# GeertRoks/AMD-Versal-phylogenetic-likelihood-function

Measured on AMD Instinct MI355X. Metric: PLF sites/sec (4-state DNA, fp64) at 1/2/4/8 MI355X; % HBM roofline, higher is better.
Workload: dtype f64

## Files before the change

amd-versal-phylogenetic-likelihood-function_amd/csrc/plf_psr.hip:

```cpp
#include <hip/hip_runtime.h>

#include <algorithm>
#include <cstdint>

#define PLFX_SECONDARY_TU
#include "plf_psr.hpp"
#include "plf_kernels.hpp"
#include "plf_launch.hpp"

namespace plfx {
namespace {

using dev::kBlock;
static_assert(kBlockThreads == kBlock, "block size mismatch");
static_assert(dev::kMaxBatch == kMaxBatch && dev::kWsWords == kWsWords, "batch constants");
using bools = among<false, true>;

template <typename T>
constexpr int kNodeU = sizeof(T) == 8 ? 2 : 4;
constexpr int kStreamU = 4;

template <typename T, bool T1, bool T2>
hipError_t launch_plf_psr_t(const NodeDescH *nodes, int count, const void *EV, const uint8_t *rate_cat, int ncat,
                            const int32_t *wgt, int64_t n, const void *tipvec, unsigned long long *ws,
                            int max_blocks, hipStream_t s) {
  constexpr int U = kNodeU<T>;
  const auto p = pack<dev::NodeBatch>(nodes, count, [](const NodeDescH &d) { return d.scaler_sum != nullptr; });
  static int cache[2] = {0, 0};
  auto go = [&](auto kSum) {
    auto kernel = &dev::plf_psr_kernel<T, U, kSum(), T1, T2>;
    const int64_t gx = grid_x((const void *)kernel, cache[kSum() ? 1 : 0], n, kBlock * U, count, max_blocks);
    return launch(kernel, dim3((unsigned)gx, (unsigned)count), kBlock, s, p.b, (const T *)EV, rate_cat, ncat, wgt,
                  n, ws, (const T *)tipvec);
  };
  return p.any_sum ? go(std::true_type{}) : go(std::false_type{});
}

template <typename T, int kTips>
hipError_t launch_plf_psr_triples_t(const TripleDescH *t, int count, const void *EV, const uint8_t *rate_cat,
                                    int ncat, const int32_t *wgt, int64_t n, const void *tipvec,
                                    unsigned long long *ws, int max_blocks, hipStream_t s) {
  constexpr int U = kNodeU<T>;
  static_assert(dev::PsrTripleLds<T, kTips>::kValues * sizeof(T) <= 160 * 1024, "LDS of a gfx950 workgroup");
  const auto p = pack<dev::TripleBatch>(t, count, [](const TripleDescH &d) { return d.ssa || d.ssb || d.ssp; });
  static int cache[2] = {0, 0};
  auto go = [&](auto kSum) {
    auto kernel = &dev::plf_psr_triple_kernel<T, U, kSum(), kTips>;
    const int64_t gx = grid_x((const void *)kernel, cache[kSum() ? 1 : 0], n, kBlock * U, count, max_blocks);
    return launch(kernel, dim3((unsigned)gx, (unsigned)count), kBlock, s, p.b, (const T *)EV, rate_cat, ncat, wgt,
                  n, ws, (const T *)tipvec);
  };
  return p.any_sum ? go(std::true_type{}) : go(std::false_type{});
}

template <typename K>
int64_t lnl_grid(K kernel, int &cache, int64_t n, int max_blocks) {
  return std::min<int64_t>(grid_x((const void *)kernel, cache, n, kBlock * kStreamU, 1, max_blocks), kLnlMaxGrid);
}

template <typename T>
int64_t edge_deriv_psr_grid(int64_t n, int max_blocks) {
  static int cache = 0;
  return lnl_grid(&dev::edge_deriv_psr_kernel<T, kStreamU>, cache, n, max_blocks);
}

template <typename T>
constexpr int kSumtabSitesPerTrip = kBlock * 4 / (4 * (int)sizeof(T) / 16);

}

hipError_t launch_plf_psr(int dtype, int tips, const NodeDescH *nodes, int count, const void *EV,
                          const uint8_t *rate_cat, int ncat, const int32_t *wgt, int64_t n, const void *tipvec,
                          unsigned long long *ws, int max_blocks, hipStream_t s) {
  if (count < 1 || count > kMaxBatch || ncat < 1 || ncat > dev::kPsrMaxCats || n < 1) return hipErrorInvalidValue;
  return dispatch(
      [&](auto k64, auto kT1, auto kT2) {
        return launch_plf_psr_t<real_t<k64()>, kT1(), kT2()>(nodes, count, EV, rate_cat, ncat, wgt, n, tipvec, ws,
                                                            max_blocks, s);
      },
      bools{dtype == 1}, bools{(tips & 1) != 0}, bools{(tips & 2) != 0});
}

hipError_t launch_plf_psr_triples(int dtype, int tips, const TripleDescH *t, int count, const void *EV,
                                  const uint8_t *rate_cat, int ncat, const int32_t *wgt, int64_t n,
                                  const void *tipvec, unsigned long long *ws, int max_blocks, hipStream_t s) {
  static_assert(dev::kMaxTriples == kMaxTriples, "triple batch size");
  if (count < 1 || count > kMaxTriples || ncat < 1 || ncat > dev::kPsrMaxCats || n < 1) return hipErrorInvalidValue;
  return dispatch(
      [&](auto k64, auto kTips) {
        return launch_plf_psr_triples_t<real_t<k64()>, kTips()>(t, count, EV, rate_cat, ncat, wgt, n, tipvec, ws,
                                                                max_blocks, s);
      },
      bools{dtype == 1}, among<0, 1, 2>{tips});
}

hipError_t launch_root_lnl_psr(int dtype, const void *x, int64_t n, const double *freq, const int32_t *wgt,
                               const int64_t *scaler_sums, int nsums, double *partials,
                               unsigned long long *ticket, double *out, double *site_lnl, int max_blocks,
                               hipStream_t s) {
  return dispatch(
      [&](auto k64) {
        using T = real_t<k64()>;
        static int cache = 0;
        auto kernel = &dev::root_lnl_psr_kernel<T, kStreamU>;
        const int64_t gx = lnl_grid(kernel, cache, n, max_blocks);
// ... 78 lines not shown
```

amd-versal-phylogenetic-likelihood-function_amd/csrc/plf_psr.hpp:

```cpp
#pragma once
#include <hip/hip_runtime.h>
#include <cstdint>
#include <type_traits>

#include "plf_edge.hpp"

namespace plfx {
namespace dev {

constexpr int kPsrMaxCats = 32;

template <typename T>
struct PsrRow {
  static constexpr int kChunk = 16 / (int)sizeof(T);
  static constexpr int kStride = 16 + kChunk;
  using V = std::conditional_t<sizeof(T) == 8, f64x2, f32x4>;
};

__device__ __forceinline__ int psr_cat(int byte, int ncat) { return byte < ncat ? byte : ncat - 1; }

template <typename T>
__device__ __forceinline__ void psr_stage(const T *__restrict__ P, int ncat, T *sP) {
  for (int i = threadIdx.x; i < ncat * 16; i += kBlock) sP[(i >> 4) * PsrRow<T>::kStride + (i & 15)] = P[i];
}

template <typename T>
__device__ __forceinline__ void psr_tip_table(const T *__restrict__ P, const T *__restrict__ tv, int ncat,
                                              T *tab) {
  for (int i = threadIdx.x; i < ncat * 64; i += kBlock) {
    const int c = i >> 6, code = (i >> 2) & 15, k = i & 3;
    T v = T(0);
#pragma unroll
    for (int l = 0; l < 4; l++) v += (tv ? tv[code * 4 + l] : T((code >> l) & 1)) * P[c * 16 + k * 4 + l];
    tab[i] = v;
  }
}

template <typename T, int N>
__device__ __forceinline__ void psr_lds_row(const T *row, T (&m)[N]) {
  using V = typename PsrRow<T>::V;
  constexpr int kChunk = PsrRow<T>::kChunk;
  static_assert(N % kChunk == 0, "whole chunks");
  const V *r = reinterpret_cast<const V *>(row);
#pragma unroll
  for (int j = 0; j < N / kChunk; j++) {
    const V v = r[j];
#pragma unroll
    for (int e = 0; e < kChunk; e++) m[j * kChunk + e] = v[e];
  }
}

template <typename T, int U, bool kSum, bool T1, bool T2>
__global__ void __launch_bounds__(kBlock)
plf_psr_kernel(const NodeBatch nodes, const T *__restrict__ EV, const uint8_t *__restrict__ rate_cat, int ncat,
               const int32_t *__restrict__ wgt, int64_t n, unsigned long long *ws,
               const T *__restrict__ tipvec) {
  constexpr int kStride = PsrRow<T>::kStride;
  const NodeDesc &d = nodes.d[blockIdx.y];
  const T *__restrict__ x1 = static_cast<const T *>(d.x1);
  const T *__restrict__ x2 = static_cast<const T *>(d.x2);
  const uint8_t *__restrict__ tip1 = static_cast<const uint8_t *>(d.x1);
  const uint8_t *__restrict__ tip2 = static_cast<const uint8_t *>(d.x2);
  T *__restrict__ x3 = static_cast<T *>(d.x3);
  uint8_t *__restrict__ scaler = d.scaler;
  unsigned long long *wsn = ws + (size_t)blockIdx.y * kWsWords;

  __shared__ __attribute__((aligned(16))) T sL[T1 ? 4 : kPsrMaxCats * kStride];
  __shared__ __attribute__((aligned(16))) T sR[T2 ? 4 : kPsrMaxCats * kStride];
  __shared__ __attribute__((aligned(16))) T tab1[T1 ? kPsrMaxCats * 64 : 4];
  __shared__ __attribute__((aligned(16))) T tab2[T2 ? kPsrMaxCats * 64 : 4];
  if constexpr (T1) psr_tip_table<T>(static_cast<const T *>(d.left), tipvec, ncat, tab1);
  else psr_stage<T>(static_cast<const T *>(d.left), ncat, sL);
  if constexpr (T2) psr_tip_table<T>(static_cast<const T *>(d.right), tipvec, ncat, tab2);
  else psr_stage<T>(static_cast<const T *>(d.right), ncat, sR);
  __syncthreads();

  T E[16];
#pragma unroll
  for (int i = 0; i < 16; i++) E[i] = EV[i];
  const T m = Num<T>::minlik();

  long long acc = 0;
  const int64_t stride = (int64_t)gridDim.x * (kBlock * U);
  const int64_t nlast = n - 1;
  for (int64_t base = (int64_t)blockIdx.x * (kBlock * U); base < n; base += stride) {
    T a[U][4], b[U][4];
    int cat[U], k1[U], k2[U], w[U];
#pragma unroll
    for (int u = 0; u < U; u++) {
      const int64_t site = base + u * kBlock + threadIdx.x;
      const int64_t ld = site < n ? site : nlast;
      cat[u] = rate_cat[ld];
      if constexpr (T1) k1[u] = tip1[ld] & 15;
      else Num<T>::template load4<true>(x1 + ld * 4, a[u]);
      if constexpr (T2) k2[u] = tip2[ld] & 15;
      else Num<T>::template load4<true>(x2 + ld * 4, b[u]);
      if (kSum) w[u] = wgt_at(wgt, ld, ws);
    }
#pragma unroll
    for (int u = 0; u < U; u++) {
      const int64_t site = base + u * kBlock + threadIdx.x;
      const int c = psr_cat(cat[u], ncat);
      T u1[4], u2[4];
      if constexpr (T1) {
        psr_lds_row<T, 4>(tab1 + (c * 16 + k1[u]) * 4, u1);
      } else {
        T PL[16];
        psr_lds_row<T, 16>(sL + c * kStride, PL);
#pragma unroll
        for (int k = 0; k < 4; k++) {
          u1[k] = T(0);
#pragma unroll
          for (int l = 0; l < 4; l++) u1[k] += a[u][l] * PL[k * 4 + l];
        }
      }
      if constexpr (T2) {
        psr_lds_row<T, 4>(tab2 + (c * 16 + k2[u]) * 4, u2);
      } else {
        T PR[16];
        psr_lds_row<T, 16>(sR + c * kStride, PR);
#pragma unroll
        for (int k = 0; k < 4; k++) {
          u2[k] = T(0);
#pragma unroll
          for (int l = 0; l < 4; l++) u2[k] += b[u][l] * PR[k * 4 + l];
        }
      }
      T o[4] = {T(0), T(0), T(0), T(0)};
#pragma unroll
      for (int k = 0; k < 4; k++) {
        const T p = u1[k] * u2[k];
#pragma unroll
        for (int l = 0; l < 4; l++) o[l] += p * E[4 * k + l];
      }
      const bool sc = (Num<T>::abs(o[0]) < m) && (Num<T>::abs(o[1]) < m) && (Num<T>::abs(o[2]) < m) &&
                      (Num<T>::abs(o[3]) < m);
#pragma unroll
// ... 46 lines not shown
    const T p = u1[k] * u2[k];
#pragma unroll
    for (int l = 0; l < 4; l++) o[l] += p * E[4 * k + l];
  }
  const bool sc = (Num<T>::abs(o[0]) < m) && (Num<T>::abs(o[1]) < m) && (Num<T>::abs(o[2]) < m) &&
                  (Num<T>::abs(o[3]) < m);
#pragma unroll
  for (int l = 0; l < 4; l++) {
    const T s = o[l] * Num<T>::two32();
    o[l] = sc ? s : o[l];
  }
  return sc;
}

template <typename T, int kTips>
struct PsrTripleLds {
  static constexpr int kMat = kPsrMaxCats * PsrRow<T>::kStride;
  static constexpr int kTab = kPsrMaxCats * 64;
  static constexpr int kSide1 = kTips >= 1 ? kTab : kMat, kSide2 = kTips == 2 ? kTab : kMat;
  static constexpr int kValues = 2 * kSide1 + 2 * kSide2 + 2 * kMat;
};

template <typename T, int U, bool kSum, int kTips>
__global__ void __launch_bounds__(kBlock)
plf_psr_triple_kernel(const TripleBatch tb, const T *__restrict__ EV, const uint8_t *__restrict__ rate_cat,
                      int ncat, const int32_t *__restrict__ wgt, int64_t n, unsigned long long *ws,
                      const T *__restrict__ tipvec) {
  constexpr bool T1 = kTips >= 1, T2 = kTips == 2;
  constexpr int kStride = PsrRow<T>::kStride;
  using Lds = PsrTripleLds<T, kTips>;
  const TripleDesc &d = tb.d[blockIdx.y];

  __shared__ __attribute__((aligned(16))) T lds[Lds::kValues];
  T *const sA1 = lds, *const sB1 = sA1 + Lds::kSide1, *const sA2 = sB1 + Lds::kSide1;
  T *const sB2 = sA2 + Lds::kSide2, *const sLP = sB2 + Lds::kSide2, *const sRP = sLP + Lds::kMat;
  if constexpr (T1) {
    psr_tip_table<T>((const T *)d.la, tipvec, ncat, sA1);
    psr_tip_table<T>((const T *)d.lb, tipvec, ncat, sB1);
  } else {
    psr_stage<T>((const T *)d.la, ncat, sA1);
    psr_stage<T>((const T *)d.lb, ncat, sB1);
  }
  if constexpr (T2) {
    psr_tip_table<T>((const T *)d.ra, tipvec, ncat, sA2);
    psr_tip_table<T>((const T *)d.rb, tipvec, ncat, sB2);
  } else {
    psr_stage<T>((const T *)d.ra, ncat, sA2);
    psr_stage<T>((const T *)d.rb, ncat, sB2);
  }
  psr_stage<T>((const T *)d.lp, ncat, sLP);
  psr_stage<T>((const T *)d.rp, ncat, sRP);
  __syncthreads();

  T E[16];
#pragma unroll
  for (int i = 0; i < 16; i++) E[i] = EV[i];
  const T m = Num<T>::minlik();
  const T *__restrict__ xa1 = (const T *)d.a1, *__restrict__ xa2 = (const T *)d.a2;
  const T *__restrict__ xb1 = (const T *)d.b1, *__restrict__ xb2 = (const T *)d.b2;
  const uint8_t *__restrict__ ta1 = (const uint8_t *)d.a1, *__restrict__ ta2 = (const uint8_t *)d.a2;
  const uint8_t *__restrict__ tb1 = (const uint8_t *)d.b1, *__restrict__ tb2 = (const uint8_t *)d.b2;
  T *__restrict__ xa = (T *)d.xa, *__restrict__ xb = (T *)d.xb, *__restrict__ xp = (T *)d.xp;

  long long accA = 0, accB = 0, accP = 0;
  const int64_t stride = (int64_t)gridDim.x * (kBlock * U);
  const int64_t nlast = n - 1;
  for (int64_t base = (int64_t)blockIdx.x * (kBlock * U); base < n; base += stride) {
    T va1[U][4], va2[U][4], vb1[U][4], vb2[U][4];
    int cat[U], ka1[U], ka2[U], kb1[U], kb2[U], w[U];
#pragma unroll
    for (int u = 0; u < U; u++) {
      const int64_t site = base + u * kBlock + threadIdx.x;
      const int64_t ld = site < n ? site : nlast;
      cat[u] = rate_cat[ld];
      if constexpr (T1) {
        ka1[u] = ta1[ld] & 15;
        kb1[u] = tb1[ld] & 15;
      } else {
        Num<T>::template load4<true>(xa1 + ld * 4, va1[u]);
        Num<T>::template load4<true>(xb1 + ld * 4, vb1[u]);
      }
      if constexpr (T2) {
        ka2[u] = ta2[ld] & 15;
        kb2[u] = tb2[ld] & 15;
      } else {
        Num<T>::template load4<true>(xa2 + ld * 4, va2[u]);
        Num<T>::template load4<true>(xb2 + ld * 4, vb2[u]);
      }
      if (kSum) w[u] = wgt_at(wgt, ld, ws);
    }
#pragma unroll
    for (int u = 0; u < U; u++) {
      const int64_t site = base + u * kBlock + threadIdx.x;
      const int c = psr_cat(cat[u], ncat);
      T oA[4], oB[4], oP[4];
      const bool sA = psr_site<T, T1, T2>(va1[u], va2[u], T1 ? sA1 + (c * 16 + ka1[u]) * 4 : sA1 + c * kStride,
                                          T2 ? sA2 + (c * 16 + ka2[u]) * 4 : sA2 + c * kStride, E, m, oA);
      const bool sB = psr_site<T, T1, T2>(vb1[u], vb2[u], T1 ? sB1 + (c * 16 + kb1[u]) * 4 : sB1 + c * kStride,
                                          T2 ? sB2 + (c * 16 + kb2[u]) * 4 : sB2 + c * kStride, E, m, oB);
      const bool sP = psr_site<T, false, false>(oA, oB, sLP + c * kStride, sRP + c * kStride, E, m, oP);
      if (site < n) {
        Num<T>::store4_nt(xa + site * 4, oA);
        Num<T>::store4_nt(xb + site * 4, oB);
        Num<T>::store4_nt(xp + site * 4, oP);
        if (d.sa) d.sa[site] = (uint8_t)sA;
        if (d.sb) d.sb[site] = (uint8_t)sB;
        if (d.sp) d.sp[site] = (uint8_t)sP;
        if (kSum) {
          accA += sA ? (long long)w[u] : 0ll;
          accB += sB ? (long long)w[u] : 0ll;
          accP += sP ? (long long)w[u] : 0ll;
        }
      }
    }
  }
  if constexpr (kSum)
    block_ticket_sum3(accA, accB, accP, ws + (size_t)blockIdx.y * 3 * kWsWords, d.ssa, d.ssb, d.ssp);
}

// ... 226 lines not shown
```

amd-versal-phylogenetic-likelihood-function_amd/csrc/plfx_api.hip:

```cpp
#include <hip/hip_runtime.h>

#include <cmath>
#include <cstdarg>
#include <cstdio>
#include <cstring>
#include <algorithm>
#include <new>
#include <string>
#include <mutex>
#include <vector>

#include "../../include/plfx.h"
#include "edge_newton.hpp"
#include "plf_kernels.hpp"
#include "psr_edge_lower.hpp"
#include "psr_lower.hpp"
#include "stream_ws.hpp"
#include "testbench.hpp"
#include "trav_lower.hpp"
#include "trav_plan.hpp"

constexpr int kHostChunksMax = 16;

using plfx::StreamWs;
using plfx::aligned16;
using plfx::clv_bytes_of;
using plfx::overlap;
constexpr int kWsPool = PLFX_WS_POOL;

struct plfx_ctx {
  int device = 0;
  hipStream_t stream = nullptr;
  int max_blocks = 0;
  int node_segments = -1;
  int streams = 1;
  int fuse = 3;
  int psr_fuse = 0;
  bool lazy_tables = false;
  plfx::WsPool wss{hipStreamPerThread};
  std::vector<void *> ws_blocks;
  uint8_t *tt_codes = nullptr;
  double *edge_buf = nullptr;
  int sched[PLFX_SCHED_COUNTS] = {};
  plfx::LaunchList lowered;
  plfx::PsrLaunchList psr_lowered;
  plfx::PsrEdgeLaunchList psr_edges_lowered;
  void *d_buf = nullptr;
  size_t d_cap = 0;
  hipStream_t d2h_stream = nullptr;
  hipEvent_t chunk_done[kHostChunksMax] = {};
  std::string err;
  mutable std::recursive_mutex mu;
};

namespace {

struct DeviceGuard {
  int prev = -1;
  explicit DeviceGuard(int dev) {
    if (hipGetDevice(&prev) != hipSuccess) prev = -1;
    if (prev != dev) (void)hipSetDevice(dev);
    else prev = -1;
  }
  ~DeviceGuard() {
    if (prev >= 0) (void)hipSetDevice(prev);
  }
  DeviceGuard(const DeviceGuard &) = delete;
  DeviceGuard &operator=(const DeviceGuard &) = delete;
};

#define PLFX_BIND(ctx)                                              \
  if (!(ctx)) return PLFX_ERR_INVALID;                              \
  std::lock_guard<std::recursive_mutex> plfx_lock_((ctx)->mu);      \
  DeviceGuard plfx_guard_((ctx)->device)

constexpr size_t kWsRegions = std::max({(size_t)plfx::kMaxBatch, (size_t)7 * plfx::kMaxSeptets,
                                        (size_t)plfx::kDeepNodes, (size_t)plfx::kDeepQueueRegion + 1});
constexpr size_t kWsBytes = kWsRegions * plfx::kWsWords * sizeof(unsigned long long);
constexpr size_t kLnlPartialBytes = 3 * (size_t)plfx::kLnlMaxGrid * sizeof(double);
constexpr size_t kEdgeBufBytes = 4 * sizeof(double);
constexpr size_t kLnlTicketBytes = plfx::kWsWords * sizeof(unsigned long long);
constexpr size_t kEdgeStateRegionBytes = (size_t)plfx::kMaxBatch * plfx::kEdgeStateBytes;

int fail(plfx_ctx *ctx, int code, const char *fmt, ...) {
  if (ctx) {
    char buf[512];
    va_list ap;
    va_start(ap, fmt);
    vsnprintf(buf, sizeof buf, fmt, ap);
    va_end(ap);
// ... 357 lines not shown
                                       c.n, tipvec, ws, ctx->max_blocks, s);
    if (e != hipSuccess) return hip_fail(ctx, e, triples ? "plf_psr level-pair launch" : "plf_psr launch");
  }
  return PLFX_OK;
}

int plan_call(plfx_ctx *ctx, const plfx_trav_op *ops, int nops, const uint8_t *const *tips, int nslots, int npmats,
              int states, int fuse, plfx::TravPlan *plan) {
  std::vector<unsigned char> tip_mask;
  if (nops > 0 && tips)
    for (int sl = 0; sl < nslots; sl++) tip_mask.push_back(tips[sl] != nullptr);
  std::string err;
  if (plfx::plan_traversal(ops, nops, nslots, npmats, tip_mask.empty() ? nullptr : tip_mask.data(), states, fuse,
                           plan, &err) != PLFX_OK)
    return fail(ctx, PLFX_ERR_INVALID, "%s", err.c_str());
  return PLFX_OK;
}

int publish_sched(plfx_ctx *ctx, const plfx::TravPlan &plan, int launches) {
  static_assert(PLFX_SCHED_COUNTS == 7, "the plan's six counts, then the launches");
  std::copy(plan.counts, plan.counts + 6, ctx->sched);
  ctx->sched[6] = launches;
  return PLFX_OK;
}

int check_sumtable_args(plfx_ctx *ctx, const uint8_t *tip1, const void *x1, const void *x2, int64_t n,
                        const void *tipvec, const void *sumtab, size_t clv_bytes) {
  if ((tip1 != nullptr) == (x1 != nullptr))
    return fail(ctx, PLFX_ERR_INVALID, "side 1 needs exactly one of tip / CLV");
  if (tip1 && !tipvec)
    return fail(ctx, PLFX_ERR_INVALID, "a coded side needs tipvec (the default 0/1 table is not in eigen coordinates)");
  if (n < 0) return fail(ctx, PLFX_ERR_INVALID, "n < 0 (%lld)", (long long)n);
  if (n == 0) return PLFX_OK;
  if (!x2 || !sumtab) return fail(ctx, PLFX_ERR_INVALID, "null CLV / sum table pointer");
  if ((x1 && !aligned16(x1)) || !aligned16(x2) || !aligned16(sumtab))
    return fail(ctx, PLFX_ERR_INVALID, "CLV pointers must be 16-byte aligned");
  if (overlap(sumtab, clv_bytes, tip1 ? (const void *)tip1 : x1, tip1 ? (size_t)n : clv_bytes) ||
      overlap(sumtab, clv_bytes, x2, clv_bytes))
    return fail(ctx, PLFX_ERR_INVALID, "sumtab may not overlap x1/x2");
  return PLFX_OK;
}

int check_sums_args(plfx_ctx *ctx, const char *who, bool required, const int64_t *scaler_sums, int nsums) {
  if (!required || nsums < 0 || (nsums > 0 && !scaler_sums))
    return fail(ctx, PLFX_ERR_INVALID, "bad %s arguments", who);
  return PLFX_OK;
}

bool env_settings(plfx_ctx *ctx) {
  if (const char *env = std::getenv("PLFX_MAX_BLOCKS")) {
    int v = std::atoi(env);
    if (v > 0) ctx->max_blocks = v;
  }
  if (const char *env = std::getenv("PLFX_FUSE")) ctx->fuse = ctx->psr_fuse = std::atoi(env);
  if (const char *env = std::getenv("PLFX_NODE_SEGMENTS")) {
    if (!std::strcmp(env, "1")) ctx->node_segments = 1;
    else if (!std::strcmp(env, "0")) ctx->node_segments = 0;
    else if (!std::strcmp(env, "-1") || !std::strcmp(env, "auto") || !*env) ctx->node_segments = -1;
    else return false;
  }
  const char *env = std::getenv("PLFX_STREAMS");
  if (env && *env) {
    static_assert(PLFX_STREAMS_MAX <= 9, "PLFX_STREAMS is parsed as one digit");
    const int v = (env[0] >= '1' && env[0] <= '0' + PLFX_STREAMS_MAX && !env[1]) ? env[0] - '0' : 0;
    if (!v) return false;
    ctx->streams = v;
  }
  return true;
}

int check_edge_args(plfx_ctx *ctx, int dtype, int states, const void *sumtab, int64_t n,
                           const double *eigen, const double *rates, int ncat) {
  if (int rc = check_dtype(ctx, dtype); rc != PLFX_OK) return rc;
  if (states != 4 && states != 20) return fail(ctx, PLFX_ERR_UNSUPPORTED, "edge: states=%d not built (4, 20)", states);
  if (ncat != 4) return fail(ctx, PLFX_ERR_UNSUPPORTED, "edge: ncat=%d not built (4)", ncat);
  if (n < 0) return fail(ctx, PLFX_ERR_INVALID, "n < 0 (%lld)", (long long)n);
  if (!eigen || !rates || (n > 0 && !sumtab)) return fail(ctx, PLFX_ERR_INVALID, "edge: null sum table / eigen / rates");
  if (!aligned16(sumtab)) return fail(ctx, PLFX_ERR_INVALID, "the sum table must be 16-byte aligned");
  return PLFX_OK;
}

int check_psr_edge_args(plfx_ctx *ctx, int dtype, const void *sumtab, int64_t n, const double *eigen,
                        const double *rates, int ncat, const uint8_t *rate_cat) {
  if (int rc = check_dtype(ctx, dtype); rc != PLFX_OK) return rc;
  if (ncat < 1 || ncat > PLFX_PSR_MAX_CATS)
    return fail(ctx, PLFX_ERR_INVALID, "psr edge: ncat=%d outside 1..%d", ncat, PLFX_PSR_MAX_CATS);
  if (n < 0) return fail(ctx, PLFX_ERR_INVALID, "n < 0 (%lld)", (long long)n);
  if (!eigen || !rates || (n > 0 && (!sumtab || !rate_cat)))
    return fail(ctx, PLFX_ERR_INVALID, "psr edge: null sum table / eigen / rates / rate_cat");
  if (!aligned16(sumtab)) return fail(ctx, PLFX_ERR_INVALID, "the sum table must be 16-byte aligned");
  return PLFX_OK;
}

template <typename Eval>
int edge_newton_loop(plfx_ctx *ctx, const char *who, double t0, double tmin, double tmax, int max_evals,
                     double *t_opt, double *out3_host, int *evals, hipStream_t s, Eval eval) {
  if (!t_opt) return fail(ctx, PLFX_ERR_INVALID, "%s: null t_opt", who);
  plfx::EdgeNewton step(t0, tmin, tmax, max_evals);
  if (!step.valid())
    return fail(ctx, PLFX_ERR_INVALID, "%s: needs 0 < tmin <= t0 <= tmax and max_evals >= 1", who);
  if (capturing(s))
    return fail(ctx, PLFX_ERR_INVALID, "%s waits for every evaluation: not on a capturing stream", who);
  double *d_t = ctx->edge_buf, *d_out = ctx->edge_buf + 1;
  double t = 0.0, out[3] = {0.0, 0.0, 0.0};
  for (bool more = true; more;) {
    t = step.t();
    PLFX_HIP(ctx, hipMemcpyAsync(d_t, &t, sizeof t, hipMemcpyHostToDevice, s));
// ... 441 lines not shown
}

int plfx_edge_optimize_dev(plfx_ctx *ctx, int dtype, int states, const void *const *sumtabs, int nedges,
                           int64_t n, const double *eigen, const double *rates, int ncat, const double *catw,
                           const int32_t *wgt, const double *t0, double tmin, double tmax, int max_evals,
                           double *t_opt, double *out3, int32_t *evals, void *stream) {
  PLFX_BIND(ctx);
  if (nedges < 1 || !sumtabs) return fail(ctx, PLFX_ERR_INVALID, "edge_optimize_dev: nedges=%d / null sumtabs", nedges);
  for (int j = 0; j < nedges; j++) {
    if (!sumtabs[j]) return fail(ctx, PLFX_ERR_INVALID, "edge_optimize_dev: sum table %d is null", j);
    if (int rc = check_edge_args(ctx, dtype, states, sumtabs[j], n, eigen, rates, ncat); rc != PLFX_OK) return rc;
  }
  if (!t0 || !t_opt) return fail(ctx, PLFX_ERR_INVALID, "edge_optimize_dev: null t0 / t_opt");
  if (!(tmin > 0.0 && tmin <= tmax && std::isfinite(tmax)) || max_evals < 1 || max_evals > PLFX_EDGE_MAX_EVALS)
    return fail(ctx, PLFX_ERR_INVALID, "edge_optimize_dev: needs 0 < tmin <= tmax < inf and 1 <= max_evals <= %d",
                PLFX_EDGE_MAX_EVALS);
  hipStream_t s = pick(stream);
  PLFX_WS(ctx, s, w);
  for (int g = 0; g < nedges; g += plfx::kMaxBatch) {
    const int c = std::min(nedges - g, plfx::kMaxBatch);
    hipError_t e = plfx::launch_edge_optimize(dtype, states, sumtabs + g, c, n, eigen, rates, catw, wgt, t0 + g, tmin,
                                              tmax, max_evals, w->edge_state, w->lnl_partials, w->ws, t_opt + g,
                                              out3 ? out3 + 3 * (size_t)g : nullptr, evals ? evals + g : nullptr,
                                              ctx->max_blocks, s);
    if (e != hipSuccess) return hip_fail(ctx, e, "edge_optimize_dev launch");
  }
  return PLFX_OK;
}


int plfx_plf_psr_dev(plfx_ctx *ctx, int dtype, const plfx_psr_node *nodes, int count, const void *EV,
                     int64_t n, const uint8_t *rate_cat, int ncat, const int32_t *wgt, const void *tipvec,
                     void *stream) {
  PLFX_BIND(ctx);
  static_assert(PLFX_PSR_MAX_CATS <= 256, "a category is one byte");
  std::string err;
  const plfx::PsrCall call{dtype, n, ncat, EV, rate_cat};
  if (plfx::lower_psr(call, nodes, count, &ctx->psr_lowered, &err) != PLFX_OK)
    return fail(ctx, PLFX_ERR_INVALID, "%s", err.c_str());
  hipStream_t s = pick(stream);
  if (n == 0) return zero_node_sums(ctx, s, nodes, count);
  PLFX_WS(ctx, s, w);
  return execute_psr(ctx, ctx->psr_lowered, call, wgt, tipvec, s, w->ws);
}

int plfx_traverse_psr(plfx_ctx *ctx, int dtype, const plfx_trav_op *ops, int nops, void *const *clv,
                      const uint8_t *const *tips, int nslots, const void *pmats, int npmats,
                      const void *EV, int64_t n, const uint8_t *rate_cat, int ncat, const int32_t *wgt,
                      uint8_t *const *scalers, int64_t *scaler_sums, const void *tipvec, void *stream) {
  PLFX_BIND(ctx);
  for (int &c : ctx->sched) c = 0;
  if (nops < 0 || (nops > 0 && (!ops || !clv))) return fail(ctx, PLFX_ERR_INVALID, "bad traverse_psr arguments");
  plfx::TravPlan plan;
  if (int rc = plan_call(ctx, ops, nops, tips, nslots, npmats, 4, std::min(ctx->psr_fuse, 1), &plan); rc != PLFX_OK)
    return rc;
  const plfx::TravArrays arrays{ops, nops, clv, tips, pmats, scalers, scaler_sums};
  const plfx::PsrCall call{dtype, n, ncat, EV, rate_cat};
  std::string err;
  if (plfx::lower_psr_traversal(plan, arrays, call, &ctx->psr_lowered, &err) != PLFX_OK)
    return fail(ctx, PLFX_ERR_INVALID, "%s", err.c_str());
  hipStream_t s = pick(stream);
  if (n == 0 || nops == 0) {
    const int rc = zero_sums(ctx, s, scaler_sums, nops);
    return rc != PLFX_OK ? rc : publish_sched(ctx, plan, 0);
  }
  PLFX_WS(ctx, s, w);
  if (int rc = execute_psr(ctx, ctx->psr_lowered, call, wgt, tipvec, s, w->ws); rc != PLFX_OK) return rc;
  return publish_sched(ctx, plan, ctx->psr_lowered.launches());
}

int plfx_root_lnl_psr(plfx_ctx *ctx, int dtype, const void *x, int64_t n, const double *freq,
                      const int32_t *wgt, const int64_t *scaler_sums, int nsums, double *out_lnl,
                      double *site_lnl, void *stream) {
  PLFX_BIND(ctx);
  if (int rc = check_dtype(ctx, dtype); rc != PLFX_OK) return rc;
  if (int rc = check_sums_args(ctx, "root_lnl_psr", out_lnl && n >= 0 && (n == 0 || x), scaler_sums, nsums);
      rc != PLFX_OK)
    return rc;
  if (!aligned16(x)) return fail(ctx, PLFX_ERR_INVALID, "the CLV must be 16-byte aligned");
  hipStream_t s = pick(stream);
  if (n == 0) {
    const int rc = zero_sums(ctx, s, out_lnl, 1);
    if (rc != PLFX_OK || nsums == 0) return rc;
  }
  PLFX_WS(ctx, s, w);
  hipError_t e = plfx::launch_root_lnl_psr(dtype, x, n, freq, wgt, scaler_sums, nsums, w->lnl_partials,
                                           w->lnl_ticket, out_lnl, site_lnl, ctx->max_blocks, s);
  if (e != hipSuccess) return hip_fail(ctx, e, "root_lnl_psr launch");
  return PLFX_OK;
}

int plfx_edge_sumtable_psr(plfx_ctx *ctx, int dtype, const uint8_t *tip1, const void *x1, const void *x2,
                           int64_t n, const void *tipvec, void *sumtab, void *stream) {
  PLFX_BIND(ctx);
  if (int rc = check_dtype(ctx, dtype); rc != PLFX_OK) return rc;
  const int rc = check_sumtable_args(ctx, tip1, x1, x2, n, tipvec, sumtab, plfx::psr_clv_bytes(dtype, n));
  if (rc != PLFX_OK || n == 0) return rc;
  hipError_t e = plfx::launch_edge_sumtable_psr(dtype, tip1 != nullptr, tip1 ? (const void *)tip1 : x1, x2, n,
                                                tipvec, sumtab, ctx->max_blocks, pick(stream));
  if (e != hipSuccess) return hip_fail(ctx, e, "edge_sumtable_psr launch");
  return PLFX_OK;
}

int plfx_edge_derivatives_psr(plfx_ctx *ctx, int dtype, const void *sumtab, int64_t n, const double *eigen,
                              const double *rates, int ncat, const uint8_t *rate_cat, const int32_t *wgt,
                              const double *t, const int64_t *scaler_sums, int nsums, double *out3,
                              double *site_lnl, void *stream) {
  PLFX_BIND(ctx);
// ... 71 lines not shown
```

amd-versal-phylogenetic-likelihood-function_amd/csrc/psr_lower.cpp:

```cpp
#include "psr_lower.hpp"

#include <algorithm>
#include <cstdint>
#include <cstdio>
#include <utility>

namespace plfx {
namespace {

struct Prefix {
  const char *call, *unit;
};
constexpr Prefix kBatch{"psr", "psr node"}, kTrav{"psr traverse", "psr traverse op"};

int refuse(PsrLaunchList *out, std::string *err, const Prefix &who, const char *what, int i = -1) {
  out->clear();
  if (err) {
    char buf[160];
    if (i >= 0) std::snprintf(buf, sizeof buf, "%s %d: %s", who.unit, i, what);
    else std::snprintf(buf, sizeof buf, "%s: %s", who.call, what);
    *err = buf;
  }
  return PLFX_ERR_INVALID;
}

const char *check_call(const PsrCall &c, const char *own, bool none, bool *run) {
  *run = false;
  if (c.dtype != PLFX_F32 && c.dtype != PLFX_F64) return "bad dtype";
  if (c.ncat < 1 || c.ncat > PLFX_PSR_MAX_CATS) return "ncat outside 1..PLFX_PSR_MAX_CATS";
  if (c.n < 0) return "n < 0";
  if (own) return own;
  if (c.n == 0 || none) return nullptr;
  if (!c.EV || !c.rate_cat) return "null EV / rate_cat";
  *run = true;
  return nullptr;
}

const char *check_node(const plfx_node &d, bool t1, bool t2, size_t cb, size_t n) {
  if (!d.x1 || !d.x2 || !d.x3 || !d.left || !d.right) return "null CLV / tip / matrix pointer";
  if ((!t1 && !aligned16(d.x1)) || (!t2 && !aligned16(d.x2)) || !aligned16(d.x3))
    return "CLV pointers must be 16-byte aligned";
  if (overlap(d.x3, cb, d.x1, t1 ? n : cb) || overlap(d.x3, cb, d.x2, t2 ? n : cb))
    return "the parent may not overlap a child it reads";
  return nullptr;
}

void add_nodes(PsrLaunchList *out, int level, const std::vector<NodeDescH> (&nb)[4]) {
  for (int k = 0; k < 4; k++) {
    const int first = (int)out->nodes.size(), count = (int)nb[k].size();
    out->nodes.insert(out->nodes.end(), nb[k].begin(), nb[k].end());
    for (int i = 0; i < count; i += kMaxBatch)
      out->items.push_back(PsrLaunch{kPsrNodes, level, k, first + i, std::min(kMaxBatch, count - i)});
  }
}

}

int lower_psr(const PsrCall &call, const plfx_psr_node *nodes, int count, PsrLaunchList *out, std::string *err) {
  out->clear();
  bool run;
  if (const char *f = check_call(call, count < 1 || !nodes ? "needs count >= 1 nodes" : nullptr, false, &run))
    return refuse(out, err, kBatch, f);
  if (!run) return PLFX_OK;

  const size_t cb = psr_clv_bytes(call.dtype, call.n);
  std::vector<NodeDescH> nb[4];
  for (int i = 0; i < count; i++) {
    const plfx_psr_node &d = nodes[i];
    if ((d.tip1 != nullptr) == (d.x1 != nullptr)) return refuse(out, err, kBatch, "child 1 needs exactly one of tip / CLV", i);
    if ((d.tip2 != nullptr) == (d.x2 != nullptr)) return refuse(out, err, kBatch, "child 2 needs exactly one of tip / CLV", i);
    const bool t1 = d.tip1 != nullptr, t2 = d.tip2 != nullptr;
    const plfx_node nd{t1 ? (const void *)d.tip1 : d.x1, t2 ? (const void *)d.tip2 : d.x2, d.x3, d.left, d.right,
                       d.scaler, d.scaler_sum};
    if (const char *f = check_node(nd, t1, t2, cb, (size_t)call.n)) return refuse(out, err, kBatch, f, i);
    nb[(t1 ? 1 : 0) | (t2 ? 2 : 0)].push_back(node_desc(nd));
  }
  add_nodes(out, 0, nb);
  return PLFX_OK;
}

int lower_psr_traversal(const TravPlan &plan, const TravArrays &t, const PsrCall &call, PsrLaunchList *out,
                        std::string *err) {
  out->clear();
  bool run;
  if (const char *f = check_call(call, t.nops < 0 || (t.nops > 0 && !t.ops) ? "null ops" : nullptr, t.nops == 0, &run))
    return refuse(out, err, kTrav, f);
  if (!run) return PLFX_OK;
  if (!t.pmats || !t.clv) return refuse(out, err, kTrav, "null pmats / clv");
  if ((int)plan.level.size() != t.nops || (int)plan.fused.size() != t.nops)
    return refuse(out, err, kTrav, "the plan is not this op list's");

  const size_t cb = psr_clv_bytes(call.dtype, call.n), tb = (size_t)call.n;
  const size_t mat_bytes = (size_t)call.ncat * 16 * (call.dtype == PLFX_F32 ? 4 : 8);
  for (int j = 0; j < t.nops; j++) {
    const OpNode d = op_node(t, mat_bytes, j);
    if (const char *f = check_node(d.nd, d.t1, d.t2, cb, tb)) return refuse(out, err, kTrav, f, j);
  }
  for (const TravGroup &g : plan.groups) {
    if (g.kind != kTravTriple || g.ops.size() != 3 || g.tips < 0 || g.tips > 2)
      return refuse(out, err, kTrav, "the plan holds a fused group other than a level pair");
    const OpNode A = op_node(t, mat_bytes, g.ops[0]), B = op_node(t, mat_bytes, g.ops[1]);
    const void *outs[3] = {A.nd.x3, B.nd.x3, t.clv[t.ops[g.ops[2]].parent]};
    const std::pair<const void *, size_t> leaves[4] = {{A.nd.x1, A.t1 ? tb : cb}, {A.nd.x2, A.t2 ? tb : cb},
                                                       {B.nd.x1, B.t1 ? tb : cb}, {B.nd.x2, B.t2 ? tb : cb}};
    for (int i = 0; i < 3; i++) {
      for (int k = i + 1; k < 3; k++)
        if (overlap(outs[i], cb, outs[k], cb))
          return refuse(out, err, kTrav, "two outputs of a fused level pair overlap", g.ops[2]);
// ... 36 lines not shown
```

amd-versal-phylogenetic-likelihood-function_amd/csrc/psr_lower.hpp:

```cpp
#pragma once
#include <string>
#include <vector>

#include "../../include/plfx.h"
#include "plf_desc.hpp"
#include "trav_lower.hpp"
#include "trav_plan.hpp"

namespace plfx {

struct PsrCall {
  int dtype;
  int64_t n;
  int ncat;
  const void *EV;
  const uint8_t *rate_cat;
};

enum PsrLaunchKind {
  kPsrNodes,
  kPsrTriples,
};

struct PsrLaunch {
  int kind;
  int level;
  int tips;
  int first, count;
};

struct PsrLaunchList {
  std::vector<PsrLaunch> items;
  std::vector<NodeDescH> nodes;
  std::vector<TripleDescH> triples;
  void clear() {
    items.clear();
    nodes.clear();
    triples.clear();
  }
  int launches() const { return (int)items.size(); }
};

inline size_t psr_clv_bytes(int dtype, int64_t n) {
  return (size_t)(n > 0 ? n : 0) * 4 * (dtype == PLFX_F32 ? 4 : 8);
}

int lower_psr(const PsrCall &call, const plfx_psr_node *nodes, int count, PsrLaunchList *out, std::string *err);

int lower_psr_traversal(const TravPlan &plan, const TravArrays &t, const PsrCall &call, PsrLaunchList *out,
                        std::string *err);

}
```

Baseline: 16.52 billion.

## Split fp64 PSR sites across lane pairs and size-gate level-pair fusion

For fp64, each site is now handled by two lanes, each owning two of the four states. Partial sums are exchanged through DPP quad moves, and loads and stores become 16-byte nontemporal vectors. Unroll and grid sizing change as well: a short-unroll variant is used when it covers n, and resident blocks per CU are capped. PSR level-pair fusion is now on by default above a site-count threshold, aiming for better coalescing, more parallelism and fewer launches, at the cost of cross-lane shuffles and a more complex launch path.

```diff
diff --git a/amd-versal-phylogenetic-likelihood-function_amd/csrc/plf_psr.hip b/amd-versal-phylogenetic-likelihood-function_amd/csrc/plf_psr.hip
--- a/amd-versal-phylogenetic-likelihood-function_amd/csrc/plf_psr.hip
+++ b/amd-versal-phylogenetic-likelihood-function_amd/csrc/plf_psr.hip
@@ -16,41 +16,57 @@
 static_assert(dev::kMaxBatch == kMaxBatch && dev::kWsWords == kWsWords, "batch constants");
 using bools = among<false, true>;
 
-template <typename T>
-constexpr int kNodeU = sizeof(T) == 8 ? 2 : 4;
+constexpr int kNodeU = 4, kTripleU = 4, kShortU = 2;
 constexpr int kStreamU = 4;
 
+template <typename T, int kLongU, bool kShort, int kPerCu, typename KernelOf, typename Batch>
+hipError_t launch_psr_stream(KernelOf kernel_of, const Packed<Batch> &p, int count, const void *EV,
+                             const uint8_t *rate_cat, int ncat, const int32_t *wgt, int64_t n, const void *tipvec,
+                             unsigned long long *ws, int max_blocks, hipStream_t s) {
+  static int cache[2][2] = {{0, 0}, {0, 0}};
+  auto with = [&](auto kSum) {
+    auto grid = [&](auto kU) {
+      const void *kernel = (const void *)kernel_of(kSum, kU);
+      int &resident = cache[kSum() ? 1 : 0][kU() == kLongU ? 0 : 1];
+      if (kPerCu > 0 && !resident)
+        resident = std::min(resident_blocks(kernel, kBlock, 2, resident), kPerCu * cu_count());
+      return grid_x(kernel, resident, n, dev::PsrMap<T>::kBlockSites * kU(), count, max_blocks);
+    };
+    auto go = [&](auto kU, int64_t gx) {
+      return launch(kernel_of(kSum, kU), dim3((unsigned)gx, (unsigned)count), kBlock, s, p.b, (const T *)EV, rate_cat,
+                    ncat, wgt, n, ws, (const T *)tipvec);
+    };
+    constexpr std::integral_constant<int, kShortU> kS{};
+    constexpr std::integral_constant<int, kLongU> kL{};
+    if constexpr (kShort) {
+      const int64_t gx = grid(kS);
+      if (gx * (dev::PsrMap<T>::kBlockSites * kShortU) >= n) return go(kS, gx);
+    }
+    return go(kL, grid(kL));
+  };
+  return p.any_sum ? with(std::true_type{}) : with(std::false_type{});
+}
+
+constexpr int kNodeBlocksPerCu64 = 3;
 template <typename T, bool T1, bool T2>
 hipError_t launch_plf_psr_t(const NodeDescH *nodes, int count, const void *EV, const uint8_t *rate_cat, int ncat,
                             const int32_t *wgt, int64_t n, const void *tipvec, unsigned long long *ws,
                             int max_blocks, hipStream_t s) {
-  constexpr int U = kNodeU<T>;
   const auto p = pack<dev::NodeBatch>(nodes, count, [](const NodeDescH &d) { return d.scaler_sum != nullptr; });
-  static int cache[2] = {0, 0};
-  auto go = [&](auto kSum) {
-    auto kernel = &dev::plf_psr_kernel<T, U, kSum(), T1, T2>;
-    const int64_t gx = grid_x((const void *)kernel, cache[kSum() ? 1 : 0], n, kBlock * U, count, max_blocks);
-    return launch(kernel, dim3((unsigned)gx, (unsigned)count), kBlock, s, p.b, (const T *)EV, rate_cat, ncat, wgt,
-                  n, ws, (const T *)tipvec);
-  };
-  return p.any_sum ? go(std::true_type{}) : go(std::false_type{});
+  return launch_psr_stream<T, kNodeU, sizeof(T) == 8, sizeof(T) == 8 ? kNodeBlocksPerCu64 : 0>(
+      [](auto kSum, auto kU) { return &dev::plf_psr_kernel<T, kU(), kSum(), T1, T2>; }, p, count, EV, rate_cat, ncat,
+      wgt, n, tipvec, ws, max_blocks, s);
 }
 
 template <typename T, int kTips>
 hipError_t launch_plf_psr_triples_t(const TripleDescH *t, int count, const void *EV, const uint8_t *rate_cat,
                                     int ncat, const int32_t *wgt, int64_t n, const void *tipvec,
                                     unsigned long long *ws, int max_blocks, hipStream_t s) {
-  constexpr int U = kNodeU<T>;
   static_assert(dev::PsrTripleLds<T, kTips>::kValues * sizeof(T) <= 160 * 1024, "LDS of a gfx950 workgroup");
   const auto p = pack<dev::TripleBatch>(t, count, [](const TripleDescH &d) { return d.ssa || d.ssb || d.ssp; });
-  static int cache[2] = {0, 0};
-  auto go = [&](auto kSum) {
-    auto kernel = &dev::plf_psr_triple_kernel<T, U, kSum(), kTips>;
-    const int64_t gx = grid_x((const void *)kernel, cache[kSum() ? 1 : 0], n, kBlock * U, count, max_blocks);
-    return launch(kernel, dim3((unsigned)gx, (unsigned)count), kBlock, s, p.b, (const T *)EV, rate_cat, ncat, wgt,
-                  n, ws, (const T *)tipvec);
-  };
-  return p.any_sum ? go(std::true_type{}) : go(std::false_type{});
+  return launch_psr_stream<T, kTripleU, true, 0>(
+      [](auto kSum, auto kU) { return &dev::plf_psr_triple_kernel<T, kU(), kSum(), kTips>; }, p, count, EV, rate_cat,
+      ncat, wgt, n, tipvec, ws, max_blocks, s);
 }
 
 template <typename K>
diff --git a/amd-versal-phylogenetic-likelihood-function_amd/csrc/plf_psr.hpp b/amd-versal-phylogenetic-likelihood-function_amd/csrc/plf_psr.hpp
--- a/amd-versal-phylogenetic-likelihood-function_amd/csrc/plf_psr.hpp
+++ b/amd-versal-phylogenetic-likelihood-function_amd/csrc/plf_psr.hpp
@@ -48,6 +48,65 @@
 #pragma unroll
     for (int e = 0; e < kChunk; e++) m[j * kChunk + e] = v[e];
   }
+}
+
+template <typename T>
+struct PsrMap {
+  static constexpr int kLanes = sizeof(T) == 8 ? 2 : 1;
+  static constexpr int kBlockSites = kBlock / kLanes;
+};
+
+constexpr int kPairSwap = 1 | (0 << 2) | (3 << 4) | (2 << 6);
+
+__device__ __forceinline__ void psr_pair_ev(const double *__restrict__ EV, int h, double (&E)[4][2]) {
+#pragma unroll
+  for (int k = 0; k < 4; k++)
+#pragma unroll
+    for (int t = 0; t < 2; t++) E[k][t] = EV[4 * k + 2 * h + t];
+}
+
+__device__ __forceinline__ void psr_pair_ump(const f64x2 x, const double *rows, double (&u)[2]) {
+  double P[8];
+  psr_lds_row<double, 8>(rows, P);
+  const double x0 = dpp_f64<kQuadEven>(x.x), x1 = dpp_f64<kQuadEven>(x.y);
+  const double x2 = dpp_f64<kQuadOdd>(x.x), x3 = dpp_f64<kQuadOdd>(x.y);
+#pragma unroll
+  for (int kk = 0; kk < 2; kk++) {
+    double v = 0.0;
+    v += x0 * P[kk * 4 + 0];
+    v += x1 * P[kk * 4 + 1];
+    v += x2 * P[kk * 4 + 2];
+    v += x3 * P[kk * 4 + 3];
+    u[kk] = v;
+  }
+}
+
+template <bool T1, bool T2>
+__device__ __forceinline__ bool psr_pair_site(const f64x2 a, const f64x2 b, const double *row1, const double *row2,
+                                              const double (&E)[4][2], double m, f64x2 &o) {
+  double u1[2], u2[2];
+  if constexpr (T1) psr_lds_row<double, 2>(row1, u1);
+  else psr_pair_ump(a, row1, u1);
+  if constexpr (T2) psr_lds_row<double, 2>(row2, u2);
+  else psr_pair_ump(b, row2, u2);
+  const double q0 = u1[0] * u2[0], q1 = u1[1] * u2[1];
+  const double p[4] = {dpp_f64<kQuadEven>(q0), dpp_f64<kQuadEven>(q1), dpp_f64<kQuadOdd>(q0), dpp_f64<kQuadOdd>(q1)};
+  double v[2];
+#pragma unroll
+  for (int t = 0; t < 2; t++) {
+    v[t] = 0.0;
+#pragma unroll
+    for (int k = 0; k < 4; k++) v[t] += p[k] * E[k][t];
+  }
+  const int small = (__builtin_fabs(v[0]) < m) && (__builtin_fabs(v[1]) < m);
+  const bool sc = (small & __builtin_amdgcn_mov_dpp(small, kPairSwap, 0xf, 0xf, true)) != 0;
+#pragma unroll
+  for (int t = 0; t < 2; t++) {
+    const double s = v[t] * Num<double>::two32();
+    v[t] = sc ? s : v[t];
+  }
+  o = f64x2{v[0], v[1]};
+  return sc;
 }
 
 template <typename T, int U, bool kSum, bool T1, bool T2>
@@ -75,14 +134,55 @@
   else psr_stage<T>(static_cast<const T *>(d.right), ncat, sR);
   __syncthreads();
 
+  const T m = Num<T>::minlik();
+  long long acc = 0;
+  const int64_t nlast = n - 1;
+  if constexpr (sizeof(T) == 8) {
+    constexpr int kSites = PsrMap<T>::kBlockSites;
+    const int h = threadIdx.x & 1, ls = threadIdx.x >> 1;
+    double E[4][2];
+    psr_pair_ev(EV, h, E);
+    const int64_t stride = (int64_t)gridDim.x * (kSites * U);
+    for (int64_t base = (int64_t)blockIdx.x * (kSites * U); base < n; base += stride) {
+      f64x2 a[U], b[U];
+      int cat[U], k1[U], k2[U], w[U];
+#pragma unroll
+      for (int u = 0; u < U; u++) {
+        const int64_t site = base + u * kSites + ls;
+        const int64_t ld = site < n ? site : nlast;
+        cat[u] = rate_cat[ld];
+        if constexpr (T1) k1[u] = tip1[ld] & 15;
+        else a[u] = __builtin_nontemporal_load(reinterpret_cast<const f64x2 *>(x1 + ld * 4) + h);
+        if constexpr (T2) k2[u] = tip2[ld] & 15;
+        else b[u] = __builtin_nontemporal_load(reinterpret_cast<const f64x2 *>(x2 + ld * 4) + h);
+        if (kSum) w[u] = wgt_at(wgt, ld, ws);
+      }
+#pragma unroll
+      for (int u = 0; u < U; u++) {
+        const int64_t site = base + u * kSites + ls;
+        const int c = psr_cat(cat[u], ncat);
+        f64x2 o;
+        const bool sc = psr_pair_site<T1, T2>(T1 ? f64x2{} : a[u], T2 ? f64x2{} : b[u],
+                                              T1 ? tab1 + (c * 16 + k1[u]) * 4 + 2 * h : sL + c * kStride + 8 * h,
+                                              T2 ? tab2 + (c * 16 + k2[u]) * 4 + 2 * h : sR + c * kStride + 8 * h, E,
+                                              m, o);
+        if (site < n) {
+          __builtin_nontemporal_store(o, reinterpret_cast<f64x2 *>(x3 + site * 4) + h);
+          if (h == 0) {
+            if (scaler) scaler[site] = (uint8_t)sc;
+            if (kSum) acc += sc ? (long long)w[u] : 0ll;
+          }
+        }
+      }
+    }
+    if constexpr (kSum) block_ticket_sum(acc, wsn, d.scaler_sum);
+    return;
+  }
+
   T E[16];
 #pragma unroll
   for (int i = 0; i < 16; i++) E[i] = EV[i];
-  const T m = Num<T>::minlik();
-
-  long long acc = 0;
   const int64_t stride = (int64_t)gridDim.x * (kBlock * U);
-  const int64_t nlast = n - 1;
   for (int64_t base = (int64_t)blockIdx.x * (kBlock * U); base < n; base += stride) {
     T a[U][4], b[U][4];
     int cat[U], k1[U], k2[U], w[U];
@@ -235,9 +335,6 @@
   psr_stage<T>((const T *)d.rp, ncat, sRP);
   __syncthreads();
 
-  T E[16];
-#pragma unroll
-  for (int i = 0; i < 16; i++) E[i] = EV[i];
   const T m = Num<T>::minlik();
   const T *__restrict__ xa1 = (const T *)d.a1, *__restrict__ xa2 = (const T *)d.a2;
   const T *__restrict__ xb1 = (const T *)d.b1, *__restrict__ xb2 = (const T *)d.b2;
@@ -246,8 +343,76 @@
   T *__restrict__ xa = (T *)d.xa, *__restrict__ xb = (T *)d.xb, *__restrict__ xp = (T *)d.xp;
 
   long long accA = 0, accB = 0, accP = 0;
+  const int64_t nlast = n - 1;
+  if constexpr (sizeof(T) == 8) {
+    constexpr int kSites = PsrMap<T>::kBlockSites;
+    const int h = threadIdx.x & 1, ls = threadIdx.x >> 1;
+    double E[4][2];
+    psr_pair_ev(EV, h, E);
+    const int64_t stride = (int64_t)gridDim.x * (kSites * U);
+    for (int64_t base = (int64_t)blockIdx.x * (kSites * U); base < n; base += stride) {
+      f64x2 va1[U], va2[U], vb1[U], vb2[U];
+      int cat[U], ka1[U], ka2[U], kb1[U], kb2[U], w[U];
+#pragma unroll
+      for (int u = 0; u < U; u++) {
+        const int64_t site = base + u * kSites + ls;
+        const int64_t ld = site < n ? site : nlast;
+        cat[u] = rate_cat[ld];
+        if constexpr (T1) {
+          ka1[u] = ta1[ld] & 15;
+          kb1[u] = tb1[ld] & 15;
+        } else {
+          va1[u] = __builtin_nontemporal_load(reinterpret_cast<const f64x2 *>(xa1 + ld * 4) + h);
+          vb1[u] = __builtin_nontemporal_load(reinterpret_cast<const f64x2 *>(xb1 + ld * 4) + h);
+        }
+        if constexpr (T2) {
+          ka2[u] = ta2[ld] & 15;
+          kb2[u] = tb2[ld] & 15;
+        } else {
+          va2[u] = __builtin_nontemporal_load(reinterpret_cast<const f64x2 *>(xa2 + ld * 4) + h);
+          vb2[u] = __builtin_nontemporal_load(reinterpret_cast<const f64x2 *>(xb2 + ld * 4) + h);
+        }
+        if (kSum) w[u] = wgt_at(wgt, ld, ws);
+      }
+#pragma unroll
+      for (int u = 0; u < U; u++) {
+        const int64_t site = base + u * kSites + ls;
+        const int c = psr_cat(cat[u], ncat);
+        const int mrow = c * kStride + 8 * h, trow = c * 64 + 2 * h;
+        f64x2 oA, oB, oP;
+        const bool sA = psr_pair_site<T1, T2>(T1 ? f64x2{} : va1[u], T2 ? f64x2{} : va2[u],
+                                              T1 ? sA1 + trow + 4 * ka1[u] : sA1 + mrow,
+                                              T2 ? sA2 + trow + 4 * ka2[u] : sA2 + mrow, E, m, oA);
+        const bool sB = psr_pair_site<T1, T2>(T1 ? f64x2{} : vb1[u], T2 ? f64x2{} : vb2[u],
+                                              T1 ? sB1 + trow + 4 * kb1[u] : sB1 + mrow,
+                                              T2 ? sB2 + trow + 4 * kb2[u] : sB2 + mrow, E, m, oB);
+        const bool sP = psr_pair_site<false, false>(oA, oB, sLP + mrow, sRP + mrow, E, m, oP);
+        if (site < n) {
+          __builtin_nontemporal_store(oA, reinterpret_cast<f64x2 *>(xa + site * 4) + h);
+          __builtin_nontemporal_store(oB, reinterpret_cast<f64x2 *>(xb + site * 4) + h);
+          __builtin_nontemporal_store(oP, reinterpret_cast<f64x2 *>(xp + site * 4) + h);
+          if (h == 0) {
+            if (d.sa) d.sa[site] = (uint8_t)sA;
+            if (d.sb) d.sb[site] = (uint8_t)sB;
+            if (d.sp) d.sp[site] = (uint8_t)sP;
+            if (kSum) {
+              accA += sA ? (long long)w[u] : 0ll;
+              accB += sB ? (long long)w[u] : 0ll;
+              accP += sP ? (long long)w[u] : 0ll;
+            }
+          }
+        }
+      }
+    }
+    if constexpr (kSum)
+      block_ticket_sum3(accA, accB, accP, ws + (size_t)blockIdx.y * 3 * kWsWords, d.ssa, d.ssb, d.ssp);
+    return;
+  }
+
+  T E[16];
+#pragma unroll
+  for (int i = 0; i < 16; i++) E[i] = EV[i];
   const int64_t stride = (int64_t)gridDim.x * (kBlock * U);
-  const int64_t nlast = n - 1;
   for (int64_t base = (int64_t)blockIdx.x * (kBlock * U); base < n; base += stride) {
     T va1[U][4], va2[U][4], vb1[U][4], vb2[U][4];
     int cat[U], ka1[U], ka2[U], kb1[U], kb2[U], w[U];
diff --git a/amd-versal-phylogenetic-likelihood-function_amd/csrc/plfx_api.hip b/amd-versal-phylogenetic-likelihood-function_amd/csrc/plfx_api.hip
--- a/amd-versal-phylogenetic-likelihood-function_amd/csrc/plfx_api.hip
+++ b/amd-versal-phylogenetic-likelihood-function_amd/csrc/plfx_api.hip
@@ -35,7 +35,7 @@
   int node_segments = -1;
   int streams = 1;
   int fuse = 3;
-  int psr_fuse = 0;
+  int psr_fuse = -1;
   bool lazy_tables = false;
   plfx::WsPool wss{hipStreamPerThread};
   std::vector<void *> ws_blocks;
@@ -499,7 +499,10 @@
     int v = std::atoi(env);
     if (v > 0) ctx->max_blocks = v;
   }
-  if (const char *env = std::getenv("PLFX_FUSE")) ctx->fuse = ctx->psr_fuse = std::atoi(env);
+  if (const char *env = std::getenv("PLFX_FUSE")) {
+    ctx->fuse = std::atoi(env);
+    ctx->psr_fuse = std::max(ctx->fuse, 0);
+  }
   if (const char *env = std::getenv("PLFX_NODE_SEGMENTS")) {
     if (!std::strcmp(env, "1")) ctx->node_segments = 1;
     else if (!std::strcmp(env, "0")) ctx->node_segments = 0;
@@ -1047,8 +1050,8 @@
   for (int &c : ctx->sched) c = 0;
   if (nops < 0 || (nops > 0 && (!ops || !clv))) return fail(ctx, PLFX_ERR_INVALID, "bad traverse_psr arguments");
   plfx::TravPlan plan;
-  if (int rc = plan_call(ctx, ops, nops, tips, nslots, npmats, 4, std::min(ctx->psr_fuse, 1), &plan); rc != PLFX_OK)
-    return rc;
+  const int fuse = plfx::psr_fuse_by_size(ctx->psr_fuse, dtype, n);
+  if (int rc = plan_call(ctx, ops, nops, tips, nslots, npmats, 4, fuse, &plan); rc != PLFX_OK) return rc;
   const plfx::TravArrays arrays{ops, nops, clv, tips, pmats, scalers, scaler_sums};
   const plfx::PsrCall call{dtype, n, ncat, EV, rate_cat};
   std::string err;
diff --git a/amd-versal-phylogenetic-likelihood-function_amd/csrc/psr_lower.cpp b/amd-versal-phylogenetic-likelihood-function_amd/csrc/psr_lower.cpp
--- a/amd-versal-phylogenetic-likelihood-function_amd/csrc/psr_lower.cpp
+++ b/amd-versal-phylogenetic-likelihood-function_amd/csrc/psr_lower.cpp
@@ -54,6 +54,11 @@
   }
 }
 
+}
+
+int psr_fuse_by_size(int setting, int dtype, int64_t n) {
+  if (setting >= 0) return setting >= 1 ? 1 : 0;
+  return n >= (dtype == PLFX_F32 ? kPsrFuseMinSitesF32 : kPsrFuseMinSitesF64) ? 1 : 0;
 }
 
 int lower_psr(const PsrCall &call, const plfx_psr_node *nodes, int count, PsrLaunchList *out, std::string *err) {
diff --git a/amd-versal-phylogenetic-likelihood-function_amd/csrc/psr_lower.hpp b/amd-versal-phylogenetic-likelihood-function_amd/csrc/psr_lower.hpp
--- a/amd-versal-phylogenetic-likelihood-function_amd/csrc/psr_lower.hpp
+++ b/amd-versal-phylogenetic-likelihood-function_amd/csrc/psr_lower.hpp
@@ -45,6 +45,10 @@
   return (size_t)(n > 0 ? n : 0) * 4 * (dtype == PLFX_F32 ? 4 : 8);
 }
 
+constexpr int64_t kPsrFuseMinSitesF64 = 1 << 16;
+constexpr int64_t kPsrFuseMinSitesF32 = 1 << 16;
+int psr_fuse_by_size(int setting, int dtype, int64_t n);
+
 int lower_psr(const PsrCall &call, const plfx_psr_node *nodes, int count, PsrLaunchList *out, std::string *err);
 
 int lower_psr_traversal(const TravPlan &plan, const TravArrays &t, const PsrCall &call, PsrLaunchList *out,
```

Measured after the change: 16.52 billion. About the same (-0.0%).
